# qc-tum/TNC

Hardware: NVIDIA H100
Metric: pairwise contractions/sec (effective ZGEMM TFLOP/s in zgemm_tflops) (higher is better)
Workload: dtype f64

## Files before the change

### tnc_b200/csrc/crt.cu

```cuda
#include "internal.h"
#include "sm90.h"
#include <cuda.h>
#include <algorithm>
#include <cmath>
#include <cstdio>
#include <cstdlib>

namespace tncb {

constexpr int CRT_MAX_MOD = 20;
static const int kModuli[CRT_MAX_MOD] = {256, 253, 251, 249, 247, 245, 241, 239, 233, 229,
                                         227, 223, 211, 199, 197, 193, 191, 181, 179, 173};
constexpr int CRT_BT = 128;
constexpr int CRT_BKB = WG_BKB;
#ifndef CRT_RING3_STAGES
#define CRT_RING3_STAGES 3
#endif
#ifndef CRT_RING3_BK
#define CRT_RING3_BK 128
#endif
#ifndef CRT_RING4_STAGES
#define CRT_RING4_STAGES 5
#endif
#ifndef CRT_RING4_BK
#define CRT_RING4_BK 64
#endif
template <bool KARA> struct CrtRing {
  static constexpr int STAGES = KARA ? CRT_RING3_STAGES : CRT_RING4_STAGES;
  static constexpr int BK = KARA ? CRT_RING3_BK : CRT_RING4_BK;
  using Stage = WgStage<KARA, BK>;
  static constexpr int SMEM = STAGES * Stage::BYTES + 1024;
  static_assert(SMEM <= 232448 - 1024, "stage ring exceeds the per-block shared memory of sm_90");
};
constexpr int CRT_KCHUNK_MAX = 32768;
constexpr int CRT_G = 34;

struct CrtTables {
  int nmod;
  int a_bits_a, a_bits_b;
  int mod[CRT_MAX_MOD];
  int magic[CRT_MAX_MOD];
  double inv_mod[CRT_MAX_MOD];
  double rho1[CRT_MAX_MOD];
  double rho2[CRT_MAX_MOD];
  double p_scaled;
};

double crt_log2_product(int n) {
  double s = 0;
  for (int i = 0; i < n; i++) s += std::log2((double)kModuli[i]);
  return s;
}

void crt_choose(long long K, int want_bits, int nmod_force, int* nmod, int* bits_a, int* bits_b) {
  const double lk = std::log2((double)std::max<long long>(K, 1));
  auto needed = [&](int bits) {
    int q = 2;
    while (q < CRT_MAX_MOD && crt_log2_product(q) - 1e-9 < 2.0 * bits + lk + 3.0) q++;
    return q;
  };
  int n = nmod_force > 0 ? std::min(nmod_force, needed(53)) : needed(want_bits);
  n = std::max(2, std::min(n, CRT_MAX_MOD));
  int tot = (int)std::floor(crt_log2_product(n) - lk - 3.0 - 1e-9);
  tot = std::max(tot, 2);
  int a = std::min(want_bits, tot / 2), b = std::min(want_bits, tot - a);
  *nmod = n; *bits_a = a; *bits_b = b;
}

int crt_bits_for_tolerance(long long K, double tol) {
  if (!(tol > 0.0)) return 53;
  const int a = (int)std::ceil(std::log2(16.0 * (double)std::max<long long>(K, 1) / tol));
  return std::max(8, std::min(53, a));
}

static void crt_make_tables(int nmod, int bits_a, int bits_b, CrtTables& T) {
  T.nmod = nmod; T.a_bits_a = bits_a; T.a_bits_b = bits_b;
  long double P = 1.0L;
  for (int i = 0; i < nmod; i++) P *= (long double)kModuli[i];
  for (int i = 0; i < CRT_MAX_MOD; i++) { T.mod[i] = 1; T.magic[i] = 0; T.inv_mod[i] = 1.0; T.rho1[i] = T.rho2[i] = 0.0; }
  for (int i = 0; i < nmod; i++) {
    const int m = kModuli[i];
    long long pim = 1;
    for (int j = 0; j < nmod; j++) if (j != i) pim = (pim * (kModuli[j] % m)) % m;
    long long inv = 1;
    while ((pim * inv) % m != 1) inv++;
    const unsigned long long num = (unsigned long long)inv << CRT_G;
    const unsigned long long q = num / (unsigned long long)m, rem = num % (unsigned long long)m;
    T.mod[i] = m;
    T.magic[i] = (int)std::llround(4294967296.0 / (double)m);
    T.inv_mod[i] = 1.0 / (double)m;
    T.rho1[i] = std::ldexp((double)q, -CRT_G);
    T.rho2[i] = std::ldexp((double)rem / (double)m, -CRT_G);
  }
  T.p_scaled = (double)std::ldexp(P, -(bits_a + bits_b));
}

int crt_export_tables(int nmod, int* moduli, double* rho1, double* rho2, double* log2_product) {
  CrtTables T;
  crt_make_tables(nmod, 0, 0, T);
  for (int i = 0; i < nmod; i++) {
    if (moduli) moduli[i] = T.mod[i];
    if (rho1) rho1[i] = T.rho1[i];
    if (rho2) rho2[i] = T.rho2[i];
  }
  if (log2_product) *log2_product = crt_log2_product(nmod);
  return TNCB_OK;
}

constexpr int RES_ROWS_C = 32, RES_K_C = 128;
constexpr int kExpNonFinite = 0x7fffffff;
constexpr int kExpMin = -1000;

__device__ __forceinline__ int crt_exp_from_bits(unsigned long long bits) {
  const int field = (int)(bits >> 52) & 0x7ff;
  if (field == 0x7ff) return kExpNonFinite;
  if (field == 0) return bits == 0ull ? 0 : kExpMin;
  return max(field - 1022, kExpMin);
}

__device__ __forceinline__ void crt_tile_coord(int e, int lk, int& r, int& k) {
  const int lane = e & 31, blk = e >> 5;
  const int kb = blk & ((128 >> lk) - 1), rb = blk >> (7 - lk);
  k = (kb << lk) + (lane & ((1 << lk) - 1));
  r = (rb << (5 - lk)) + (lane >> lk);
}

__global__ void __launch_bounds__(256)
crt_rowmax_kernel(const double2* __restrict__ src, const long long* __restrict__ off_row, const long long* __restrict__ off_k,
                  long long rows, long long K, int lk, unsigned long long* __restrict__ rowmax) {
  __shared__ unsigned long long s_max[RES_ROWS_C];
  __shared__ long long s_offr[RES_ROWS_C], s_offk[RES_K_C];
  const long long row0 = (long long)blockIdx.x * RES_ROWS_C, k0 = (long long)blockIdx.y * RES_K_C;
  const int tid = threadIdx.x;
  if (tid < RES_ROWS_C) { s_max[tid] = 0ull; s_offr[tid] = row0 + tid < rows ? __ldg(off_row + row0 + tid) : -1; }
  else if (tid >= 128) { const int k = tid - 128; s_offk[k] = k0 + k < K ? __ldg(off_k + k0 + k) : -1; }
  __syncthreads();
  unsigned long long mv[RES_ROWS_C * RES_K_C / 256];
#pragma unroll
  for (int it = 0; it < RES_ROWS_C * RES_K_C / 256; it++) {
    int r, k;
    crt_tile_coord(it * 256 + tid, lk, r, k);
    const long long orow = s_offr[r], ok = s_offk[k];
    mv[it] = 0ull;
    if (orow >= 0 && ok >= 0) {
      const double2 v = __ldg(src + orow + ok);
      mv[it] = max((unsigned long long)__double_as_longlong(fabs(v.x)), (unsigned long long)__double_as_longlong(fabs(v.y)));
    }
  }
  int cur_r = -1;
  unsigned long long cur_m = 0ull;
#pragma unroll
  for (int it = 0; it < RES_ROWS_C * RES_K_C / 256; it++) {
    int r, k;
    crt_tile_coord(it * 256 + tid, lk, r, k);
    unsigned long long m = mv[it];
    for (int d = 1; d < (1 << lk); d <<= 1) m = max(m, __shfl_xor_sync(0xffffffffu, m, d));
    if (r != cur_r) {
      if (cur_m && (tid & ((1 << lk) - 1)) == 0) atomicMax(&s_max[cur_r], cur_m);
      cur_r = r; cur_m = 0ull;
    }
    cur_m = max(cur_m, m);
  }
  if (cur_m && (tid & ((1 << lk) - 1)) == 0) atomicMax(&s_max[cur_r], cur_m);
  __syncthreads();
  if (tid < RES_ROWS_C && row0 + tid < rows && s_max[tid] != 0ull) atomicMax(rowmax + row0 + tid, s_max[tid]);
}

__device__ __forceinline__ int crt_fix_byte(int s, int m) {
  if (s > 127) s -= m;
  else if (s < -128) s += m;
  return s;
}
constexpr int RES_ROWS = RES_ROWS_C, RES_K = RES_K_C, RES_RS = RES_K + RES_K / 8 + 1;
template <int COMPS, bool KARA>
__global__ void __launch_bounds__(256, 3)
crt_residue_kernel(const double2* __restrict__ src, const long long* __restrict__ off_row, const long long* __restrict__ off_k,
                   long long rows, long long K, long long rowsP, long long Kp, const unsigned long long* __restrict__ rowmax, int bits, int lk,
                   const __grid_constant__ CrtTables T, int8_t* __restrict__ planes) {
  extern __shared__ __align__(16) unsigned char res_smem_raw[];
  double2* tile = reinterpret_cast<double2*>(res_smem_raw);
  __shared__ double s_scale[RES_ROWS];
  __shared__ long long s_offr[RES_ROWS], s_offk[RES_K];
  __shared__ double s_inv[CRT_MAX_MOD];
  __shared__ int s_mod[CRT_MAX_MOD];
  const long long row0 = (long long)blockIdx.x * RES_ROWS, k0 = (long long)blockIdx.y * RES_K;
  const int tid = threadIdx.x;
  const double two_a = scalbn(1.0, bits);
  if (tid >= 64 && tid < 64 + CRT_MAX_MOD) { s_inv[tid - 64] = T.inv_mod[tid - 64]; s_mod[tid - 64] = T.mod[tid - 64]; }
  if (tid < RES_ROWS) {
    const long long r = row0 + tid;
    const int e = r < rows ? crt_exp_from_bits(rowmax[r]) : 0;
    s_scale[tid] = (e == kExpNonFinite) ? 0.0 : scalbn(1.0, -e);
    s_offr[tid] = r < rows ? __ldg(off_row + r) : -1;
  } else if (tid >= 128) {
    const int k = tid - 128;
    s_offk[k] = k0 + k < K ? __ldg(off_k + k0 + k) : -1;
  }
  __syncthreads();
  double2 vv[RES_ROWS * RES_K / 256];
#pragma unroll
  for (int it = 0; it < RES_ROWS * RES_K / 256; it++) {
    int r, k;
    crt_tile_coord(it * 256 + tid, lk, r, k);
    const long long orow = s_offr[r], ok = s_offk[k];
    vv[it] = make_double2(0.0, 0.0);
    if (orow >= 0 && ok >= 0) vv[it] = __ldg(src + orow + ok);
  }
#pragma unroll
  for (int it = 0; it < RES_ROWS * RES_K / 256; it++) {
    int r, k;
    crt_tile_coord(it * 256 + tid, lk, r, k);
    const double sc = s_scale[r];
    double2 v = vv[it];
    v.x = trunc(v.x * sc * two_a);
    v.y = trunc(v.y * sc * two_a);
    if (sc == 0.0) { v.x = 0.0; v.y = 0.0; }
    tile[r * RES_RS + k + (k >> 3)] = v;
  }
  __syncthreads();
  const int r = tid >> 3;
  if (row0 + r >= rows) return;
  const double RMAGIC = 6755399441055744.0;
  const long long plane_stride = rowsP * Kp;
#pragma unroll 1
  for (int pass = 0; pass < 2; pass++) {
    const int g = (tid & 7) + 8 * pass;
    double xr[8], xi[8];
    int lr[8], li[8];
#pragma unroll
    for (int j = 0; j < 8; j++) {
      const double2 v = tile[r * RES_RS + g * 9 + j];
      xr[j] = v.x; xi[j] = v.y;
      lr[j] = (int)__double2ll_rn(v.x); li[j] = (int)__double2ll_rn(v.y);
    }
    int8_t* dst = planes + (row0 + r) * Kp + k0 + g * 8;
    const int nmod = T.nmod;
#pragma unroll 1
    for (int i = 0; i < nmod; i++) {
      const int m = s_mod[i];
      const double inv = s_inv[i];
      uint32_t wr[2] = {0, 0}, wi[2] = {0, 0}, ws[2] = {0, 0};
#pragma unroll
      for (int j = 0; j < 8; j++) {
        const int qr = __double2loint(fma(xr[j], inv, RMAGIC));
        const int qi = __double2loint(fma(xi[j], inv, RMAGIC));
        const int rr = lr[j] - qr * m, ri = li[j] - qi * m;
        constexpr uint32_t sel[4] = {0x3214u, 0x3240u, 0x3410u, 0x4210u};
        wr[j >> 2] = __byte_perm(wr[j >> 2], (uint32_t)rr, sel[j & 3]);
        wi[j >> 2] = __byte_perm(wi[j >> 2], (uint32_t)ri, sel[j & 3]);
        if (KARA) ws[j >> 2] = __byte_perm(ws[j >> 2], (uint32_t)crt_fix_byte(rr + ri, m), sel[j & 3]);
      }
      int8_t* d = dst + (long long)i * (KARA ? 3 : COMPS) * plane_stride;
      if (KARA) {
        *reinterpret_cast<uint2*>(d) = make_uint2(wr[0], wr[1]);
        *reinterpret_cast<uint2*>(d + plane_stride) = make_uint2(wi[0], wi[1]);
        *reinterpret_cast<uint2*>(d + 2 * plane_stride) = make_uint2(ws[0], ws[1]);
      } else if (COMPS == 2) {
        *reinterpret_cast<uint2*>(d) = make_uint2(wr[0], wr[1]);
        *reinterpret_cast<uint2*>(d + plane_stride) = make_uint2(wi[0], wi[1]);
      } else {
        *reinterpret_cast<uint2*>(d) = make_uint2(__vneg4(wi[0]), __vneg4(wi[1]));
        *reinterpret_cast<uint2*>(d + plane_stride) = make_uint2(wr[0], wr[1]);
        *reinterpret_cast<uint2*>(d + 2 * plane_stride) = make_uint2(wi[0], wi[1]);
      }
    }
  }
}

struct CrtGemmArgs {
  int8_t* R;
  int Np, Mp;
  int tiles_n, tiles_m, tile_m;
  int nmod, nkc, kb_per_chunk, num_kb;
  int total_items;
  int group;
  int negmod[CRT_MAX_MOD];
  int magic[CRT_MAX_MOD];
};

struct CrtItem { int mod_i, prod, kc, n0, m0; };
template <bool KARA>
__device__ __forceinline__ CrtItem crt_decode(const CrtGemmArgs& p, int item) {
  const int tiles = p.tiles_n * p.tiles_m;
  const int mk = item / tiles, t = item - mk * tiles;
  CrtItem it;
  const int mp = mk / p.nkc;
  it.kc = mk - mp * p.nkc;
  it.mod_i = KARA ? mp / 3 : mp; it.prod = KARA ? mp - it.mod_i * 3 : 0;
  const int per_band = p.group * p.tiles_m;
  const int band = t / per_band, first = band * p.group;
  const int gsize = min(p.group, p.tiles_n - first);
  const int r = t - band * per_band;
  it.n0 = (first + r % gsize) * CRT_BT;
  it.m0 = (r / gsize) * p.tile_m;
  return it;
}

template <bool KARA>
__global__ void __launch_bounds__(WG_THREADS, 1)
crt_gemm_kernel(const __grid_constant__ CUtensorMap mapB, const __grid_constant__ CUtensorMap mapA,
                const __grid_constant__ CrtGemmArgs p) {
  constexpr int STAGES = CrtRing<KARA>::STAGES, BK = CrtRing<KARA>::BK, SUB = CRT_BKB / BK;
  using Stage = typename CrtRing<KARA>::Stage;
  extern __shared__ __align__(1024) uint8_t crt_smem_raw[];
  uint8_t* smem = reinterpret_cast<uint8_t*>((reinterpret_cast<uintptr_t>(crt_smem_raw) + 1023) & ~(uintptr_t)1023);
  __shared__ uint64_t full_bar[STAGES], empty_bar[STAGES];
  const int wg = threadIdx.x >> 7, tid = threadIdx.x & 127;

  if (threadIdx.x == 0) {
    for (int s = 0; s < STAGES; s++) { wg_mbar_init(&full_bar[s], 1); wg_mbar_init(&empty_bar[s], 2); }
    asm volatile("fence.mbarrier_init.release.cluster;" ::: "memory");
  }
  __syncthreads();

  if (wg == 0) {
    wg_setmaxnreg_producer();
    if (tid != 0) return;
    int it = 0;
    for (int item = blockIdx.x; item < p.total_items; item += gridDim.x) {
      const CrtItem w = crt_decode<KARA>(p, item);
      const int kb0 = w.kc * p.kb_per_chunk, kb1 = min(p.num_kb, kb0 + p.kb_per_chunk);
      const int rowB = (KARA ? w.mod_i * 3 + w.prod : w.mod_i * 2) * p.Np + w.n0;
      const int rowA = (KARA ? w.mod_i * 3 + w.prod : w.mod_i * 3) * p.Mp + w.m0;
      for (int ks = kb0 * SUB; ks < kb1 * SUB; ks++, it++) {
        uint8_t* st = wg_produce_begin<STAGES, KARA, BK>(smem, full_bar, empty_bar, it);
        uint64_t* bar = &full_bar[it % STAGES];
        const int kx = ks * BK;
        uint8_t* a = st + Stage::A;
        wg_tma_2d(&mapB, bar, st, kx, rowB);
        if (KARA) {
          wg_tma_2d(&mapA, bar, a, kx, rowA);
          wg_tma_2d(&mapA, bar, a + Stage::TILE, kx, rowA + WG_ROWS);
        } else {
          wg_tma_2d(&mapB, bar, st + Stage::B1, kx, rowB + p.Np);
          wg_tma_2d(&mapA, bar, a, kx, rowA);
          wg_tma_2d(&mapA, bar, a + Stage::TILE, kx, rowA + p.Mp);
          wg_tma_2d(&mapA, bar, a + 2 * Stage::TILE, kx, rowA + 2 * p.Mp);
        }
      }
    }
  } else {
    wg_setmaxnreg_consumer();
    const int c = wg - 1, wq = tid >> 5, lane = tid & 31;
    const int q = lane & 3;
    const bool q0 = q & 1, q1 = q & 2;
    WgRing<STAGES, KARA, BK> ring{smem, full_bar, empty_bar};
    uint32_t acc[128];
#pragma unroll
    for (int i = 0; i < 128; i++) acc[i] = 0u;
    for (int item = blockIdx.x; item < p.total_items; item += gridDim.x) {
      const CrtItem w = crt_decode<KARA>(p, item);
      const int kb0 = w.kc * p.kb_per_chunk, kb1 = min(p.num_kb, kb0 + p.kb_per_chunk);
      bool first = true;
      for (int ks = kb0 * SUB; ks < kb1 * SUB; ks++) ring.mma_stage(acc, c, first, tid == 0);
      ring.drain(tid == 0);
      const int negm = p.negmod[w.mod_i], magic = p.magic[w.mod_i];
      int8_t* row_base[2];
#pragma unroll
      for (int h = 0; h < 2; h++) {
        const long long n = (long long)w.n0 + c * 64 + wq * 16 + (lane >> 2) + 8 * h;
        row_base[h] = KARA ? p.R + ((long long)((w.mod_i * p.nkc + w.kc) * 3 + w.prod) * p.Np + n) * p.Mp + w.m0
                           : p.R + ((long long)((w.mod_i * p.nkc + w.kc) * 2) * p.Np + n) * p.Mp + w.m0;
      }
#pragma unroll
      for (int i = 0; i < 4; i++) {
#pragma unroll
        for (int h = 0; h < 2; h++) {
          uint32_t x[4];
#pragma unroll
          for (int k = 0; k < 4; k++) {
            uint32_t u = 0;
#pragma unroll
            for (int jj = 0; jj < 2; jj++) {
#pragma unroll
              for (int e = 0; e < 2; e++) {
                const int a = (int)acc[4 * (8 * i + 2 * k + jj) + 2 * h + e];
                int t = __mulhi(a, magic) * negm + a;
                if (t > 127) t += negm;
                u |= (((uint32_t)t & 0xffu) ^ 0x80u) << (8 * (2 * jj + e));
              }
            }
            x[k] = u;
          }
          const uint32_t r0 = __shfl_xor_sync(0xffffffffu, q0 ? x[0] : x[1], 1);
          const uint32_t r1 = __shfl_xor_sync(0xffffffffu, q0 ? x[2] : x[3], 1);
          const uint32_t a0 = q0 ? r0 : x[0], a1 = q0 ? x[1] : r0;
          const uint32_t b0 = q0 ? r1 : x[2], b1 = q0 ? x[3] : r1;
          const uint32_t g0 = __shfl_xor_sync(0xffffffffu, q1 ? a0 : b0, 2);
          const uint32_t g1 = __shfl_xor_sync(0xffffffffu, q1 ? a1 : b1, 2);
          const uint32_t k0 = q1 ? b0 : a0, k1 = q1 ? b1 : a1;
          const uint32_t y0 = q1 ? g0 : k0, y1 = q1 ? g1 : k1, y2 = q1 ? k0 : g0, y3 = q1 ? k1 : g1;
          const uint4 v = make_uint4(__byte_perm(y0, y1, 0x5410), __byte_perm(y2, y3, 0x5410),
                                     __byte_perm(y0, y1, 0x7632), __byte_perm(y2, y3, 0x7632));
          const int cc = 4 * i + q;
          int8_t* dst = KARA ? row_base[h] + cc * 16
                             : row_base[h] + (i >= 2 ? (long long)p.Np * p.Mp : 0LL) + (cc & 7) * 16;
          *reinterpret_cast<uint4*>(dst) = v;
        }
      }
    }
  }
}

struct CrtReconArgs {
  const int8_t* R;
  double2* C;
  const unsigned long long* max_n;
  const unsigned long long* max_m;
  long long rows, cols, ldc;
  long long Np, Mp;
  int nkc;
};

template <bool ONE_CHUNK, bool KARA>
__global__ void __launch_bounds__(256, 4)
crt_reconstruct_kernel(const __grid_constant__ CrtReconArgs a, const __grid_constant__ CrtTables T) {
  const long long cols4 = a.Mp >> 2;
  const long long idx = (long long)blockIdx.x * blockDim.x + threadIdx.x;
  const long long n = idx / cols4, m4 = (idx - n * cols4) * 4;
  if (n >= a.rows || m4 >= a.cols) return;
  double s1r[4], s2r[4], s1i[4], s2i[4];
#pragma unroll
  for (int j = 0; j < 4; j++) { s1r[j] = s2r[j] = s1i[j] = s2i[j] = 0.0; }
  const long long plane = a.Np * a.Mp;
  const int8_t* base = a.R + n * a.Mp + m4;
  const double bias = 4503599627370496.0 + (KARA ? 256.0 : 128.0) * (double)a.nkc;
  const double bias_i = 4503599627370496.0 + (KARA ? 384.0 : 128.0) * (double)a.nkc;
#pragma unroll 8
  for (int i = 0; i < T.nmod; i++) {
    uint32_t ur[4], ui[4];
    if (KARA) {
#pragma unroll
      for (int j = 0; j < 4; j++) { ur[j] = 0; ui[j] = 0; }
      for (int c = 0; c < (ONE_CHUNK ? 1 : a.nkc); c++) {
        const int8_t* pk = base + (long long)((i * a.nkc + c) * 3) * plane;
        const uint32_t w1 = __ldg(reinterpret_cast<const uint32_t*>(pk));
        const uint32_t w2 = __ldg(reinterpret_cast<const uint32_t*>(pk + plane));
        const uint32_t w3 = __ldg(reinterpret_cast<const uint32_t*>(pk + 2 * plane));
#pragma unroll
        for (int j = 0; j < 4; j++) {
          const uint32_t k1 = __byte_perm(w1, 0, 0x4440 + j), k2 = __byte_perm(w2, 0, 0x4440 + j);
          ur[j] += 256u + k1 - k2;
          ui[j] += 512u + __byte_perm(w3, 0, 0x4440 + j) - k1 - k2;
        }
      }
    } else if (ONE_CHUNK) {
      const uint32_t wr = __ldg(reinterpret_cast<const uint32_t*>(base + (long long)(i * 2) * plane));
      const uint32_t wi = __ldg(reinterpret_cast<const uint32_t*>(base + (long long)(i * 2 + 1) * plane));
#pragma unroll
      for (int j = 0; j < 4; j++) { ur[j] = __byte_perm(wr, 0, 0x4440 + j); ui[j] = __byte_perm(wi, 0, 0x4440 + j); }
    } else {
#pragma unroll
      for (int j = 0; j < 4; j++) { ur[j] = 0; ui[j] = 0; }
      for (int c = 0; c < a.nkc; c++) {
        const int8_t* pr = base + (long long)((i * a.nkc + c) * 2) * plane;
        const uint32_t wr = __ldg(reinterpret_cast<const uint32_t*>(pr));
        const uint32_t wi = __ldg(reinterpret_cast<const uint32_t*>(pr + plane));
#pragma unroll
        for (int j = 0; j < 4; j++) { ur[j] += __byte_perm(wr, 0, 0x4440 + j); ui[j] += __byte_perm(wi, 0, 0x4440 + j); }
      }
    }
    const double r1 = T.rho1[i], r2 = T.rho2[i];
#pragma unroll
    for (int j = 0; j < 4; j++) {
      const double dr = __hiloint2double(0x43300000, (int)ur[j]) - bias;
      const double di = __hiloint2double(0x43300000, (int)ui[j]) - bias_i;
      s1r[j] = fma(dr, r1, s1r[j]); s2r[j] = fma(dr, r2, s2r[j]);
      s1i[j] = fma(di, r1, s1i[j]); s2i[j] = fma(di, r2, s2i[j]);
    }
  }
  const int en = crt_exp_from_bits(a.max_n[n]);
  double2* dst = a.C + n * a.ldc + m4;
  const double RMAGIC = 6755399441055744.0;
#pragma unroll
  for (int j = 0; j < 4; j++) {
    if (m4 + j >= a.cols) break;
    const int em = crt_exp_from_bits(a.max_m[m4 + j]);
    double2 out;
    if (en == kExpNonFinite || em == kExpNonFinite) {
      out = make_double2(__longlong_as_double(0x7ff8000000000000LL), __longlong_as_double(0x7ff8000000000000LL));
    } else {
      const double qr = ((s1r[j] + s2r[j]) + RMAGIC) - RMAGIC;
      const double qi = ((s1i[j] + s2i[j]) + RMAGIC) - RMAGIC;
      const double fr = (s1r[j] - qr) + s2r[j], fi = (s1i[j] - qi) + s2i[j];
      out = make_double2(scalbn(fr * T.p_scaled, en + em), scalbn(fi * T.p_scaled, en + em));
    }
    dst[j] = out;
  }
}

typedef CUresult (*EncodeTiledFn)(CUtensorMap*, CUtensorMapDataType, cuuint32_t, void*, const cuuint64_t*, const cuuint64_t*,
                                  const cuuint32_t*, const cuuint32_t*, CUtensorMapInterleave, CUtensorMapSwizzle,
                                  CUtensorMapL2promotion, CUtensorMapFloatOOBfill);
static EncodeTiledFn get_encode() {
  static EncodeTiledFn fn = nullptr;
  static bool tried = false;
  if (!tried) {
    tried = true;
    cudaDriverEntryPointQueryResult q;
    void* p = nullptr;
    if (cudaGetDriverEntryPoint("cuTensorMapEncodeTiled", &p, cudaEnableDefault, &q) == cudaSuccess) fn = (EncodeTiledFn)p;
  }
  return fn;
}
template <int BK>
int wg_make_map(CUtensorMap* m, void* ptr, uint64_t rows, uint64_t kbytes) {
  static_assert(BK == 128 || BK == 64, "SWIZZLE_128B or SWIZZLE_64B");
  EncodeTiledFn enc = get_encode();
  if (!enc) return fail(TNCB_ERR_CUDA, "cuTensorMapEncodeTiled is not available");
  cuuint64_t dims[2] = {kbytes, rows};
  cuuint64_t strides[1] = {kbytes};
  cuuint32_t box[2] = {(cuuint32_t)BK, (cuuint32_t)WG_ROWS};
  cuuint32_t estr[2] = {1, 1};
  CUresult r = enc(m, CU_TENSOR_MAP_DATA_TYPE_UINT8, 2, ptr, dims, strides, box, estr, CU_TENSOR_MAP_INTERLEAVE_NONE,
                   BK == 128 ? CU_TENSOR_MAP_SWIZZLE_128B : CU_TENSOR_MAP_SWIZZLE_64B, CU_TENSOR_MAP_L2_PROMOTION_L2_256B,
                   CU_TENSOR_MAP_FLOAT_OOB_FILL_NONE);
  if (r != CUDA_SUCCESS) return fail(TNCB_ERR_CUDA, "cuTensorMapEncodeTiled failed: " + std::to_string((int)r));
  return TNCB_OK;
}
template int wg_make_map<128>(CUtensorMap*, void*, uint64_t, uint64_t);
template int wg_make_map<64>(CUtensorMap*, void*, uint64_t, uint64_t);

static inline long long round_up_ll(long long x, long long a) { return (x + a - 1) / a * a; }


int launch_k1_crt(tncb_ctx* ctx, const PairPlan& P, const double2* A, const double2* B, double2* C,
                  const long long* offAm, const long long* offBn, const long long* offAk, const long long* offBk) {
  int nmod, bits_a, bits_b;
  const int want = ctx->crt_tol > 0.0 ? crt_bits_for_tolerance(P.K, ctx->crt_tol) : ctx->crt_bits;
  crt_choose(P.K, want, ctx->crt_nmod_force, &nmod, &bits_a, &bits_b);
  CrtTables T;
  crt_make_tables(nmod, bits_a, bits_b, T);
  cudaStream_t st = ctx->stream;
  const long long Kp = round_up_ll(P.K, CRT_BKB);
  const int num_kb = (int)(Kp / CRT_BKB);
  const int ctas_max = std::max(1, ctx->sm_count);
  const bool kara = ctx->crt_products == 3 || (ctx->crt_products == 0 && Kp >= ctx->crt_kara_min_k);
  const int TM = kara ? 2 * CRT_BT : CRT_BT;
  const int NPB = kara ? 3 : 2, NPR = kara ? 3 : 2;
  const long long tiles_total = round_up_ll(P.N, CRT_BT) / CRT_BT * (round_up_ll(P.M, TM) / TM);
  int nkc = (int)((Kp + CRT_KCHUNK_MAX - 1) / CRT_KCHUNK_MAX);
  {
    const long long items = tiles_total * nmod * (kara ? 3 : 1);
    const long long want = ctas_max;
    if (items * nkc < want) nkc = (int)std::min<long long>((want + items - 1) / items, std::max(1, num_kb / 8));
    nkc = std::max(1, std::min(nkc, 32));
  }
  int kb_per_chunk = (num_kb + nkc - 1) / nkc;
  nkc = (num_kb + kb_per_chunk - 1) / kb_per_chunk;
  if ((long long)kb_per_chunk * CRT_BKB > CRT_KCHUNK_MAX) return fail(TNCB_ERR_UNSUPPORTED, "K too long for the int8 engine");

  const size_t budget = ctx->crt_ws_bytes;
  long long pn = round_up_ll(P.N, CRT_BT), pm = round_up_ll(P.M, TM);
  auto ws_bytes = [&](long long n_, long long m_) {
    return (size_t)nmod * (size_t)Kp * (size_t)(NPB * n_ + 3 * m_) + (size_t)nmod * nkc * NPR * (size_t)n_ * (size_t)m_;
  };
  while (ws_bytes(pn, pm) > budget && (pm > TM || pn > CRT_BT)) {
    if (pm >= pn && pm > TM) pm = round_up_ll(pm / 2, TM);
    else if (pn > CRT_BT) pn = round_up_ll(pn / 2, CRT_BT);
    else pm = round_up_ll(pm / 2, TM);
  }
  const size_t bytesB = (size_t)nmod * NPB * pn * Kp, bytesA = (size_t)nmod * 3 * pm * Kp;
  const size_t bytesR = (size_t)nmod * nkc * NPR * pn * pm;
  const size_t bytesE = (size_t)(pn + pm) * sizeof(unsigned long long);
  void *pb = nullptr, *pa = nullptr, *pr = nullptr, *pe = nullptr;
  int rc;
  if ((rc = ctx->arena.alloc(bytesB, &pb))) return rc;
  if ((rc = ctx->arena.alloc(bytesA, &pa))) { ctx->arena.free(pb, bytesB); return rc; }
  if ((rc = ctx->arena.alloc(bytesR, &pr))) { ctx->arena.free(pb, bytesB); ctx->arena.free(pa, bytesA); return rc; }
  if ((rc = ctx->arena.alloc(bytesE, &pe))) { ctx->arena.free(pb, bytesB); ctx->arena.free(pa, bytesA); ctx->arena.free(pr, bytesR); return rc; }
  auto cleanup = [&]() { ctx->arena.free(pb, bytesB); ctx->arena.free(pa, bytesA); ctx->arena.free(pr, bytesR); ctx->arena.free(pe, bytesE); };
  unsigned long long* max_n = (unsigned long long*)pe;
  unsigned long long* max_m = max_n + pn;

  static bool attr_done_dev[64] = {false};
  bool& attr_done = attr_done_dev[ctx->device & 63];
  const int smem_gemm4 = CrtRing<false>::SMEM, smem_gemm3 = CrtRing<true>::SMEM;
  const int smem_res = RES_ROWS * RES_RS * (int)sizeof(double2);
  if (!attr_done) {
    cudaError_t e = cudaFuncSetAttribute(crt_gemm_kernel<false>, cudaFuncAttributeMaxDynamicSharedMemorySize, smem_gemm4);
    if (e == cudaSuccess) e = cudaFuncSetAttribute(crt_gemm_kernel<true>, cudaFuncAttributeMaxDynamicSharedMemorySize, smem_gemm3);
    if (e == cudaSuccess) e = cudaFuncSetAttribute(crt_residue_kernel<2, false>, cudaFuncAttributeMaxDynamicSharedMemorySize, smem_res);
    if (e == cudaSuccess) e = cudaFuncSetAttribute(crt_residue_kernel<3, false>, cudaFuncAttributeMaxDynamicSharedMemorySize, smem_res);
    if (e == cudaSuccess) e = cudaFuncSetAttribute(crt_residue_kernel<2, true>, cudaFuncAttributeMaxDynamicSharedMemorySize, smem_res);
    if (e == cudaSuccess) e = cudaFuncSetAttribute(crt_residue_kernel<3, true>, cudaFuncAttributeMaxDynamicSharedMemorySize, smem_res);
    if (e != cudaSuccess) { cleanup(); return fail(TNCB_ERR_CUDA, cudaGetErrorString(e)); }
    attr_done = true;
  }
  auto lane_split = [](const LegList& kl, bool k_is_b, const LegList& fl) {
    auto p2 = [](long long d) { int b = 0; while ((2LL << b) <= d && b < 5) b++; return b; };
    const long long ks = kl.n ? (k_is_b ? kl.sb[kl.n - 1] : kl.sa[kl.n - 1]) : (1LL << 62);
    const long long fs = fl.n ? fl.sa[fl.n - 1] : (1LL << 62);
    if (ks <= fs) return kl.n ? p2(kl.dim[kl.n - 1]) : 0;
    return 0;
  };
  const int lk_b = lane_split(P.k, true, P.n), lk_a = lane_split(P.k, false, P.m);
  ctx->last_int8_ops = 0.0; ctx->last_nmod = nmod; ctx->last_products = kara ? 3 : 4;
  bool timed = false;

  for (long long n0 = 0; n0 < P.N; n0 += pn) {
    const long long nrows = std::min(pn, P.N - n0);
    const long long Np = round_up_ll(nrows, CRT_BT);
    if (Np != nrows) cudaMemsetAsync(pb, 0, (size_t)nmod * NPB * Np * Kp, st);
    cudaMemsetAsync(max_n, 0, (size_t)nrows * sizeof(unsigned long long), st);
    {
      dim3 g((unsigned)((nrows + RES_ROWS - 1) / RES_ROWS), (unsigned)(Kp / RES_K));
      crt_rowmax_kernel<<<g, 256, 0, st>>>(B, offBn + n0, offBk, nrows, P.K, lk_b, max_n);
      if (kara) crt_residue_kernel<2, true><<<g, 256, smem_res, st>>>(B, offBn + n0, offBk, nrows, P.K, Np, Kp, max_n, bits_b, lk_b, T, (int8_t*)pb);
      else crt_residue_kernel<2, false><<<g, 256, smem_res, st>>>(B, offBn + n0, offBk, nrows, P.K, Np, Kp, max_n, bits_b, lk_b, T, (int8_t*)pb);
    }
    ctx->launches += 2;
    CUtensorMap mapB;
    if ((rc = kara ? wg_make_map<CrtRing<true>::BK>(&mapB, pb, (uint64_t)nmod * NPB * Np, (uint64_t)Kp)
                   : wg_make_map<CrtRing<false>::BK>(&mapB, pb, (uint64_t)nmod * NPB * Np, (uint64_t)Kp))) { cleanup(); return rc; }
    for (long long m0 = 0; m0 < P.M; m0 += pm) {
      const long long mcols = std::min(pm, P.M - m0);
      const long long Mp = round_up_ll(mcols, TM);
      if (Mp != mcols) cudaMemsetAsync(pa, 0, (size_t)nmod * 3 * Mp * Kp, st);
      cudaMemsetAsync(max_m, 0, (size_t)mcols * sizeof(unsigned long long), st);
      {
        dim3 g((unsigned)((mcols + RES_ROWS - 1) / RES_ROWS), (unsigned)(Kp / RES_K));
        crt_rowmax_kernel<<<g, 256, 0, st>>>(A, offAm + m0, offAk, mcols, P.K, lk_a, max_m);
        if (kara) crt_residue_kernel<3, true><<<g, 256, smem_res, st>>>(A, offAm + m0, offAk, mcols, P.K, Mp, Kp, max_m, bits_a, lk_a, T, (int8_t*)pa);
        else crt_residue_kernel<3, false><<<g, 256, smem_res, st>>>(A, offAm + m0, offAk, mcols, P.K, Mp, Kp, max_m, bits_a, lk_a, T, (int8_t*)pa);
      }
      ctx->launches += 2;
      CUtensorMap mapA;
      if ((rc = kara ? wg_make_map<CrtRing<true>::BK>(&mapA, pa, (uint64_t)nmod * 3 * Mp, (uint64_t)Kp)
                     : wg_make_map<CrtRing<false>::BK>(&mapA, pa, (uint64_t)nmod * 3 * Mp, (uint64_t)Kp))) { cleanup(); return rc; }
      CrtGemmArgs g;
      g.R = (int8_t*)pr; g.Np = (int)Np; g.Mp = (int)Mp;
      g.tiles_n = (int)(Np / CRT_BT); g.tiles_m = (int)(Mp / TM); g.tile_m = TM;
      g.nmod = nmod; g.nkc = nkc; g.kb_per_chunk = kb_per_chunk; g.num_kb = num_kb;
      const long long items = (long long)g.tiles_n * g.tiles_m * nmod * nkc * (kara ? 3 : 1);
      if (items > 0x7fffffffLL) { cleanup(); return fail(TNCB_ERR_UNSUPPORTED, "too many work items"); }
      g.total_items = (int)items;
      g.group = ctx->crt_group;
      for (int i = 0; i < CRT_MAX_MOD; i++) { g.negmod[i] = -T.mod[i]; g.magic[i] = T.magic[i]; }
      const unsigned grid = (unsigned)std::min<long long>(ctas_max, items);
      const double ops = 2.0 * (kara ? 3.0 : 4.0) * (double)nmod * (double)Np * (double)Mp * (double)Kp;
      const bool time_this = ctx->time_gemm == 2 || (ctx->time_gemm == 1 && !timed);
      if (time_this) gemm_timer_begin(ctx);
      if (kara) crt_gemm_kernel<true><<<grid, WG_THREADS, smem_gemm3, st>>>(mapB, mapA, g);
      else crt_gemm_kernel<false><<<grid, WG_THREADS, smem_gemm4, st>>>(mapB, mapA, g);
      cudaError_t e = cudaGetLastError();
      if (time_this) { gemm_timer_end(ctx, ops); timed = true; }
      if (e != cudaSuccess) { cleanup(); return fail(TNCB_ERR_CUDA, std::string("crt_gemm_kernel launch: ") + cudaGetErrorString(e)); }
      ctx->last_int8_ops += ops;
      CrtReconArgs r;
      r.R = (const int8_t*)pr; r.C = C + n0 * P.M + m0; r.max_n = max_n; r.max_m = max_m;
      r.rows = nrows; r.cols = mcols; r.ldc = P.M; r.Np = Np; r.Mp = Mp; r.nkc = nkc;
      const long long threads = nrows * (Mp / 4);
      const unsigned rg = (unsigned)((threads + 255) / 256);
      if (kara) {
        if (nkc == 1) crt_reconstruct_kernel<true, true><<<rg, 256, 0, st>>>(r, T);
        else crt_reconstruct_kernel<false, true><<<rg, 256, 0, st>>>(r, T);
      } else {
        if (nkc == 1) crt_reconstruct_kernel<true, false><<<rg, 256, 0, st>>>(r, T);
        else crt_reconstruct_kernel<false, false><<<rg, 256, 0, st>>>(r, T);
      }
      ctx->launches += 2;
    }
  }
  ctx->engine_count[4]++;
  cudaError_t e = cudaGetLastError();
  cleanup();
  if (e != cudaSuccess) return fail(TNCB_ERR_CUDA, std::string("K1' (CRT) launch: ") + cudaGetErrorString(e));
  return TNCB_OK;
}

}
```

Baseline: 5853.

## Restructure CRT residue and reconstruct kernels with cp.async staging and wider stores

The residue kernel now stages an 8x512 input tile into shared memory with cp.async, and each thread handles 16 consecutive k elements so residues go out as 16-byte stores instead of 8-byte ones. It also drops the padding memsets by covering the whole padded row range, and walks k tiles in reverse order. The single-chunk reconstruct kernel now stages each row segment's residue planes into shared memory with cp.async before decoding, in place of scattered __ldg loads. The changes aim to cut memory-transaction overhead in the pre- and post-processing around the int8 GEMM, at the cost of more shared memory per block and lower occupancy.

```diff
diff --git a/tnc_b200/csrc/crt.cu b/tnc_b200/csrc/crt.cu
--- a/tnc_b200/csrc/crt.cu
+++ b/tnc_b200/csrc/crt.cu
@@ -171,98 +171,109 @@
   else if (s < -128) s += m;
   return s;
 }
-constexpr int RES_ROWS = RES_ROWS_C, RES_K = RES_K_C, RES_RS = RES_K + RES_K / 8 + 1;
+constexpr int RES_R = 8, RES_KT = 512, RES_THREADS = 256;
+constexpr int RES_RS = RES_KT + RES_KT / 16 + 4;
+constexpr int RES_SMEM = RES_R * RES_RS * (int)sizeof(double2);
+
+static __device__ __forceinline__ void crt_cp_async16(unsigned smem_addr, const void* gptr, bool pred) {
+  asm volatile("cp.async.cg.shared.global [%0], [%1], 16, %2;\n" ::"r"(smem_addr), "l"(gptr), "r"(pred ? 16 : 0));
+}
+
 template <int COMPS, bool KARA>
-__global__ void __launch_bounds__(256, 3)
+__global__ void __launch_bounds__(RES_THREADS, 2)
 crt_residue_kernel(const double2* __restrict__ src, const long long* __restrict__ off_row, const long long* __restrict__ off_k,
-                   long long rows, long long K, long long rowsP, long long Kp, const unsigned long long* __restrict__ rowmax, int bits, int lk,
-                   const __grid_constant__ CrtTables T, int8_t* __restrict__ planes) {
+                   long long rows, long long K, long long rowsP, long long Kp, const unsigned long long* __restrict__ rowmax, int bits,
+                   int lk, const __grid_constant__ CrtTables T, int8_t* __restrict__ planes) {
   extern __shared__ __align__(16) unsigned char res_smem_raw[];
   double2* tile = reinterpret_cast<double2*>(res_smem_raw);
-  __shared__ double s_scale[RES_ROWS];
-  __shared__ long long s_offr[RES_ROWS], s_offk[RES_K];
+  __shared__ long long s_offr[RES_R], s_offk[RES_KT];
+  __shared__ double s_scale[RES_R];
   __shared__ double s_inv[CRT_MAX_MOD];
   __shared__ int s_mod[CRT_MAX_MOD];
-  const long long row0 = (long long)blockIdx.x * RES_ROWS, k0 = (long long)blockIdx.y * RES_K;
-  const int tid = threadIdx.x;
-  const double two_a = scalbn(1.0, bits);
-  if (tid >= 64 && tid < 64 + CRT_MAX_MOD) { s_inv[tid - 64] = T.inv_mod[tid - 64]; s_mod[tid - 64] = T.mod[tid - 64]; }
-  if (tid < RES_ROWS) {
+  const long long row0 = (long long)blockIdx.x * RES_R, k0 = (long long)(gridDim.y - 1 - blockIdx.y) * RES_KT;
+  const int tid = threadIdx.x, warp = tid >> 5, lane = tid & 31;
+  if (tid < CRT_MAX_MOD) { s_inv[tid] = T.inv_mod[tid]; s_mod[tid] = T.mod[tid]; }
+  if (tid < RES_R) {
     const long long r = row0 + tid;
     const int e = r < rows ? crt_exp_from_bits(rowmax[r]) : 0;
     s_scale[tid] = (e == kExpNonFinite) ? 0.0 : scalbn(1.0, -e);
     s_offr[tid] = r < rows ? __ldg(off_row + r) : -1;
-  } else if (tid >= 128) {
-    const int k = tid - 128;
-    s_offk[k] = k0 + k < K ? __ldg(off_k + k0 + k) : -1;
-  }
+  }
+  for (int k = tid; k < RES_KT; k += RES_THREADS) s_offk[k] = k0 + k < K ? __ldg(off_k + k0 + k) : -1;
   __syncthreads();
-  double2 vv[RES_ROWS * RES_K / 256];
-#pragma unroll
-  for (int it = 0; it < RES_ROWS * RES_K / 256; it++) {
-    int r, k;
-    crt_tile_coord(it * 256 + tid, lk, r, k);
-    const long long orow = s_offr[r], ok = s_offk[k];
-    vv[it] = make_double2(0.0, 0.0);
-    if (orow >= 0 && ok >= 0) vv[it] = __ldg(src + orow + ok);
-  }
-#pragma unroll
-  for (int it = 0; it < RES_ROWS * RES_K / 256; it++) {
-    int r, k;
-    crt_tile_coord(it * 256 + tid, lk, r, k);
-    const double sc = s_scale[r];
-    double2 v = vv[it];
-    v.x = trunc(v.x * sc * two_a);
-    v.y = trunc(v.y * sc * two_a);
-    if (sc == 0.0) { v.x = 0.0; v.y = 0.0; }
-    tile[r * RES_RS + k + (k >> 3)] = v;
+  {
+    const int lq = max(lk, 2);
+    const unsigned sbase = (unsigned)__cvta_generic_to_shared(tile);
+#pragma unroll
+    for (int it = 0; it < RES_R * RES_KT / RES_THREADS; it++) {
+      const int e = it * RES_THREADS + tid, blk = e >> 5;
+      const int kb = blk & ((RES_KT >> lq) - 1), rb = blk >> (9 - lq);
+      const int k = (kb << lq) + (lane & ((1 << lq) - 1)), r = (rb << (5 - lq)) + (lane >> lq);
+      const long long orow = s_offr[r], ok = s_offk[k];
+      const bool valid = orow >= 0 && ok >= 0;
+      crt_cp_async16(sbase + (unsigned)(r * RES_RS + k + (k >> 4)) * 16u, valid ? src + orow + ok : src, valid);
+    }
+    asm volatile("cp.async.commit_group;\ncp.async.wait_group 0;\n" ::: "memory");
   }
   __syncthreads();
-  const int r = tid >> 3;
-  if (row0 + r >= rows) return;
-  const double RMAGIC = 6755399441055744.0;
-  const long long plane_stride = rowsP * Kp;
-#pragma unroll 1
-  for (int pass = 0; pass < 2; pass++) {
-    const int g = (tid & 7) + 8 * pass;
-    double xr[8], xi[8];
-    int lr[8], li[8];
-#pragma unroll
-    for (int j = 0; j < 8; j++) {
-      const double2 v = tile[r * RES_RS + g * 9 + j];
-      xr[j] = v.x; xi[j] = v.y;
-      lr[j] = (int)__double2ll_rn(v.x); li[j] = (int)__double2ll_rn(v.y);
-    }
-    int8_t* dst = planes + (row0 + r) * Kp + k0 + g * 8;
+  const int r = warp, kl = lane * 16;
+  double2 v[16];
+#pragma unroll
+  for (int j = 0; j < 16; j++) v[j] = tile[r * RES_RS + kl + lane + j];
+  const double sc = s_scale[r];
+  const double two_a = scalbn(1.0, bits);
+  double xr[16], xi[16];
+  int lr[16], li[16];
+#pragma unroll
+  for (int j = 0; j < 16; j++) {
+    double2 w = v[j];
+    w.x = trunc(w.x * sc * two_a);
+    w.y = trunc(w.y * sc * two_a);
+    if (sc == 0.0) { w.x = 0.0; w.y = 0.0; }
+    xr[j] = w.x; xi[j] = w.y;
+    lr[j] = (int)__double2ll_rn(w.x); li[j] = (int)__double2ll_rn(w.y);
+  }
+  const long long kk = k0 + kl;
+  if (kk < Kp) {
+    const double RMAGIC = 6755399441055744.0;
+    const long long plane_stride = rowsP * Kp;
+    int8_t* dst = planes + (row0 + r) * Kp + kk;
     const int nmod = T.nmod;
 #pragma unroll 1
     for (int i = 0; i < nmod; i++) {
-      const int m = s_mod[i];
+      const int md = s_mod[i];
       const double inv = s_inv[i];
-      uint32_t wr[2] = {0, 0}, wi[2] = {0, 0}, ws[2] = {0, 0};
-#pragma unroll
-      for (int j = 0; j < 8; j++) {
+      uint32_t wr[4] = {0, 0, 0, 0}, wi[4] = {0, 0, 0, 0};
+#pragma unroll
+      for (int j = 0; j < 16; j++) {
         const int qr = __double2loint(fma(xr[j], inv, RMAGIC));
         const int qi = __double2loint(fma(xi[j], inv, RMAGIC));
-        const int rr = lr[j] - qr * m, ri = li[j] - qi * m;
+        const int rr = lr[j] - qr * md, ri = li[j] - qi * md;
         constexpr uint32_t sel[4] = {0x3214u, 0x3240u, 0x3410u, 0x4210u};
         wr[j >> 2] = __byte_perm(wr[j >> 2], (uint32_t)rr, sel[j & 3]);
         wi[j >> 2] = __byte_perm(wi[j >> 2], (uint32_t)ri, sel[j & 3]);
-        if (KARA) ws[j >> 2] = __byte_perm(ws[j >> 2], (uint32_t)crt_fix_byte(rr + ri, m), sel[j & 3]);
       }
-      int8_t* d = dst + (long long)i * (KARA ? 3 : COMPS) * plane_stride;
+      int8_t* d = dst;
       if (KARA) {
-        *reinterpret_cast<uint2*>(d) = make_uint2(wr[0], wr[1]);
-        *reinterpret_cast<uint2*>(d + plane_stride) = make_uint2(wi[0], wi[1]);
-        *reinterpret_cast<uint2*>(d + 2 * plane_stride) = make_uint2(ws[0], ws[1]);
+        *reinterpret_cast<uint4*>(d) = make_uint4(wr[0], wr[1], wr[2], wr[3]);
+        *reinterpret_cast<uint4*>(d + plane_stride) = make_uint4(wi[0], wi[1], wi[2], wi[3]);
+        uint32_t ws[4] = {0, 0, 0, 0};
+#pragma unroll
+        for (int j = 0; j < 16; j++) {
+          const int rr = (int)(int8_t)(wr[j >> 2] >> (8 * (j & 3))), ri = (int)(int8_t)(wi[j >> 2] >> (8 * (j & 3)));
+          constexpr uint32_t sel[4] = {0x3214u, 0x3240u, 0x3410u, 0x4210u};
+          ws[j >> 2] = __byte_perm(ws[j >> 2], (uint32_t)crt_fix_byte(rr + ri, md), sel[j & 3]);
+        }
+        *reinterpret_cast<uint4*>(d + 2 * plane_stride) = make_uint4(ws[0], ws[1], ws[2], ws[3]);
       } else if (COMPS == 2) {
-        *reinterpret_cast<uint2*>(d) = make_uint2(wr[0], wr[1]);
-        *reinterpret_cast<uint2*>(d + plane_stride) = make_uint2(wi[0], wi[1]);
+        *reinterpret_cast<uint4*>(d) = make_uint4(wr[0], wr[1], wr[2], wr[3]);
+        *reinterpret_cast<uint4*>(d + plane_stride) = make_uint4(wi[0], wi[1], wi[2], wi[3]);
       } else {
-        *reinterpret_cast<uint2*>(d) = make_uint2(__vneg4(wi[0]), __vneg4(wi[1]));
-        *reinterpret_cast<uint2*>(d + plane_stride) = make_uint2(wr[0], wr[1]);
-        *reinterpret_cast<uint2*>(d + 2 * plane_stride) = make_uint2(wi[0], wi[1]);
+        *reinterpret_cast<uint4*>(d) = make_uint4(__vneg4(wi[0]), __vneg4(wi[1]), __vneg4(wi[2]), __vneg4(wi[3]));
+        *reinterpret_cast<uint4*>(d + plane_stride) = make_uint4(wr[0], wr[1], wr[2], wr[3]);
+        *reinterpret_cast<uint4*>(d + 2 * plane_stride) = make_uint4(wi[0], wi[1], wi[2], wi[3]);
       }
+      dst += (KARA ? 3 : COMPS) * plane_stride;
     }
   }
 }
@@ -412,18 +423,46 @@
   int nkc;
 };
 
+constexpr int RECON_THREADS = 256, RECON_SEG = 4 * RECON_THREADS;
 template <bool ONE_CHUNK, bool KARA>
-__global__ void __launch_bounds__(256, 4)
+__global__ void __launch_bounds__(RECON_THREADS, 4)
 crt_reconstruct_kernel(const __grid_constant__ CrtReconArgs a, const __grid_constant__ CrtTables T) {
-  const long long cols4 = a.Mp >> 2;
-  const long long idx = (long long)blockIdx.x * blockDim.x + threadIdx.x;
-  const long long n = idx / cols4, m4 = (idx - n * cols4) * 4;
-  if (n >= a.rows || m4 >= a.cols) return;
+  extern __shared__ __align__(16) unsigned char rec_smem[];
+  long long n, m4, plane;
+  const int8_t* base;
+  if (ONE_CHUNK) {
+    const long long segs = (a.cols + RECON_SEG - 1) / RECON_SEG;
+    n = blockIdx.x / segs;
+    const long long m0 = (blockIdx.x - n * segs) * RECON_SEG;
+    const int cpr = (int)(min((long long)RECON_SEG, a.cols - m0) + 15) >> 4;
+    const int nruns = T.nmod * (KARA ? 3 : 2);
+    const int8_t* g = a.R + n * a.Mp + m0;
+    const long long gplane = a.Np * a.Mp;
+    const unsigned sbase = (unsigned)__cvta_generic_to_shared(rec_smem);
+    for (int c = threadIdx.x; c < nruns * cpr; c += RECON_THREADS) {
+      const int p = c / cpr, o = (c - p * cpr) * 16;
+      crt_cp_async16(sbase + (unsigned)(p * RECON_SEG + o), g + p * gplane + o, true);
+    }
+    asm volatile("cp.async.commit_group;\ncp.async.wait_group 0;\n" ::: "memory");
+    __syncthreads();
+    m4 = m0 + 4 * threadIdx.x;
+    if (m4 >= a.cols) return;
+    base = reinterpret_cast<const int8_t*>(rec_smem) + 4 * threadIdx.x;
+    plane = RECON_SEG;
+  } else {
+    const long long cols4 = a.Mp >> 2;
+    const long long idx = (long long)blockIdx.x * blockDim.x + threadIdx.x;
+    n = idx / cols4; m4 = (idx - n * cols4) * 4;
+    if (n >= a.rows || m4 >= a.cols) return;
+    base = a.R + n * a.Mp + m4;
+    plane = a.Np * a.Mp;
+  }
+  auto ld = [&](const int8_t* p) {
+    return ONE_CHUNK ? *reinterpret_cast<const uint32_t*>(p) : __ldg(reinterpret_cast<const uint32_t*>(p));
+  };
   double s1r[4], s2r[4], s1i[4], s2i[4];
 #pragma unroll
   for (int j = 0; j < 4; j++) { s1r[j] = s2r[j] = s1i[j] = s2i[j] = 0.0; }
-  const long long plane = a.Np * a.Mp;
-  const int8_t* base = a.R + n * a.Mp + m4;
   const double bias = 4503599627370496.0 + (KARA ? 256.0 : 128.0) * (double)a.nkc;
   const double bias_i = 4503599627370496.0 + (KARA ? 384.0 : 128.0) * (double)a.nkc;
 #pragma unroll 8
@@ -434,9 +473,7 @@
       for (int j = 0; j < 4; j++) { ur[j] = 0; ui[j] = 0; }
       for (int c = 0; c < (ONE_CHUNK ? 1 : a.nkc); c++) {
         const int8_t* pk = base + (long long)((i * a.nkc + c) * 3) * plane;
-        const uint32_t w1 = __ldg(reinterpret_cast<const uint32_t*>(pk));
-        const uint32_t w2 = __ldg(reinterpret_cast<const uint32_t*>(pk + plane));
-        const uint32_t w3 = __ldg(reinterpret_cast<const uint32_t*>(pk + 2 * plane));
+        const uint32_t w1 = ld(pk), w2 = ld(pk + plane), w3 = ld(pk + 2 * plane);
 #pragma unroll
         for (int j = 0; j < 4; j++) {
           const uint32_t k1 = __byte_perm(w1, 0, 0x4440 + j), k2 = __byte_perm(w2, 0, 0x4440 + j);
@@ -445,8 +482,7 @@
         }
       }
     } else if (ONE_CHUNK) {
-      const uint32_t wr = __ldg(reinterpret_cast<const uint32_t*>(base + (long long)(i * 2) * plane));
-      const uint32_t wi = __ldg(reinterpret_cast<const uint32_t*>(base + (long long)(i * 2 + 1) * plane));
+      const uint32_t wr = ld(base + (long long)(i * 2) * plane), wi = ld(base + (long long)(i * 2 + 1) * plane);
 #pragma unroll
       for (int j = 0; j < 4; j++) { ur[j] = __byte_perm(wr, 0, 0x4440 + j); ui[j] = __byte_perm(wi, 0, 0x4440 + j); }
     } else {
@@ -576,14 +612,15 @@
   static bool attr_done_dev[64] = {false};
   bool& attr_done = attr_done_dev[ctx->device & 63];
   const int smem_gemm4 = CrtRing<false>::SMEM, smem_gemm3 = CrtRing<true>::SMEM;
-  const int smem_res = RES_ROWS * RES_RS * (int)sizeof(double2);
   if (!attr_done) {
     cudaError_t e = cudaFuncSetAttribute(crt_gemm_kernel<false>, cudaFuncAttributeMaxDynamicSharedMemorySize, smem_gemm4);
     if (e == cudaSuccess) e = cudaFuncSetAttribute(crt_gemm_kernel<true>, cudaFuncAttributeMaxDynamicSharedMemorySize, smem_gemm3);
-    if (e == cudaSuccess) e = cudaFuncSetAttribute(crt_residue_kernel<2, false>, cudaFuncAttributeMaxDynamicSharedMemorySize, smem_res);
-    if (e == cudaSuccess) e = cudaFuncSetAttribute(crt_residue_kernel<3, false>, cudaFuncAttributeMaxDynamicSharedMemorySize, smem_res);
-    if (e == cudaSuccess) e = cudaFuncSetAttribute(crt_residue_kernel<2, true>, cudaFuncAttributeMaxDynamicSharedMemorySize, smem_res);
-    if (e == cudaSuccess) e = cudaFuncSetAttribute(crt_residue_kernel<3, true>, cudaFuncAttributeMaxDynamicSharedMemorySize, smem_res);
+    if (e == cudaSuccess) e = cudaFuncSetAttribute(crt_residue_kernel<2, false>, cudaFuncAttributeMaxDynamicSharedMemorySize, RES_SMEM);
+    if (e == cudaSuccess) e = cudaFuncSetAttribute(crt_residue_kernel<3, false>, cudaFuncAttributeMaxDynamicSharedMemorySize, RES_SMEM);
+    if (e == cudaSuccess) e = cudaFuncSetAttribute(crt_residue_kernel<2, true>, cudaFuncAttributeMaxDynamicSharedMemorySize, RES_SMEM);
+    if (e == cudaSuccess) e = cudaFuncSetAttribute(crt_residue_kernel<3, true>, cudaFuncAttributeMaxDynamicSharedMemorySize, RES_SMEM);
+    if (e == cudaSuccess) e = cudaFuncSetAttribute(crt_reconstruct_kernel<true, false>, cudaFuncAttributeMaxDynamicSharedMemorySize, CRT_MAX_MOD * 2 * RECON_SEG);
+    if (e == cudaSuccess) e = cudaFuncSetAttribute(crt_reconstruct_kernel<true, true>, cudaFuncAttributeMaxDynamicSharedMemorySize, CRT_MAX_MOD * 3 * RECON_SEG);
     if (e != cudaSuccess) { cleanup(); return fail(TNCB_ERR_CUDA, cudaGetErrorString(e)); }
     attr_done = true;
   }
@@ -595,36 +632,32 @@
     return 0;
   };
   const int lk_b = lane_split(P.k, true, P.n), lk_a = lane_split(P.k, false, P.m);
+  auto prepare = [&](const double2* src, const long long* off_row, const long long* off_k, long long rows, long long rowsP,
+                     int bits, int lk, unsigned long long* rowmax, int8_t* planes, bool bt) {
+    cudaMemsetAsync(rowmax, 0, (size_t)rows * sizeof(unsigned long long), st);
+    crt_rowmax_kernel<<<dim3((unsigned)((rows + RES_ROWS_C - 1) / RES_ROWS_C), (unsigned)(Kp / RES_K_C)), 256, 0, st>>>(
+        src, off_row, off_k, rows, P.K, lk, rowmax);
+    const dim3 g((unsigned)(rowsP / RES_R), (unsigned)((Kp + RES_KT - 1) / RES_KT));
+    if (kara && bt) crt_residue_kernel<2, true><<<g, RES_THREADS, RES_SMEM, st>>>(src, off_row, off_k, rows, P.K, rowsP, Kp, rowmax, bits, lk, T, planes);
+    else if (kara) crt_residue_kernel<3, true><<<g, RES_THREADS, RES_SMEM, st>>>(src, off_row, off_k, rows, P.K, rowsP, Kp, rowmax, bits, lk, T, planes);
+    else if (bt) crt_residue_kernel<2, false><<<g, RES_THREADS, RES_SMEM, st>>>(src, off_row, off_k, rows, P.K, rowsP, Kp, rowmax, bits, lk, T, planes);
+    else crt_residue_kernel<3, false><<<g, RES_THREADS, RES_SMEM, st>>>(src, off_row, off_k, rows, P.K, rowsP, Kp, rowmax, bits, lk, T, planes);
+    ctx->launches += 2;
+  };
   ctx->last_int8_ops = 0.0; ctx->last_nmod = nmod; ctx->last_products = kara ? 3 : 4;
   bool timed = false;
 
   for (long long n0 = 0; n0 < P.N; n0 += pn) {
     const long long nrows = std::min(pn, P.N - n0);
     const long long Np = round_up_ll(nrows, CRT_BT);
-    if (Np != nrows) cudaMemsetAsync(pb, 0, (size_t)nmod * NPB * Np * Kp, st);
-    cudaMemsetAsync(max_n, 0, (size_t)nrows * sizeof(unsigned long long), st);
-    {
-      dim3 g((unsigned)((nrows + RES_ROWS - 1) / RES_ROWS), (unsigned)(Kp / RES_K));
-      crt_rowmax_kernel<<<g, 256, 0, st>>>(B, offBn + n0, offBk, nrows, P.K, lk_b, max_n);
-      if (kara) crt_residue_kernel<2, true><<<g, 256, smem_res, st>>>(B, offBn + n0, offBk, nrows, P.K, Np, Kp, max_n, bits_b, lk_b, T, (int8_t*)pb);
-      else crt_residue_kernel<2, false><<<g, 256, smem_res, st>>>(B, offBn + n0, offBk, nrows, P.K, Np, Kp, max_n, bits_b, lk_b, T, (int8_t*)pb);
-    }
-    ctx->launches += 2;
+    prepare(B, offBn + n0, offBk, nrows, Np, bits_b, lk_b, max_n, (int8_t*)pb, true);
     CUtensorMap mapB;
     if ((rc = kara ? wg_make_map<CrtRing<true>::BK>(&mapB, pb, (uint64_t)nmod * NPB * Np, (uint64_t)Kp)
                    : wg_make_map<CrtRing<false>::BK>(&mapB, pb, (uint64_t)nmod * NPB * Np, (uint64_t)Kp))) { cleanup(); return rc; }
     for (long long m0 = 0; m0 < P.M; m0 += pm) {
       const long long mcols = std::min(pm, P.M - m0);
       const long long Mp = round_up_ll(mcols, TM);
-      if (Mp != mcols) cudaMemsetAsync(pa, 0, (size_t)nmod * 3 * Mp * Kp, st);
-      cudaMemsetAsync(max_m, 0, (size_t)mcols * sizeof(unsigned long long), st);
-      {
-        dim3 g((unsigned)((mcols + RES_ROWS - 1) / RES_ROWS), (unsigned)(Kp / RES_K));
-        crt_rowmax_kernel<<<g, 256, 0, st>>>(A, offAm + m0, offAk, mcols, P.K, lk_a, max_m);
-        if (kara) crt_residue_kernel<3, true><<<g, 256, smem_res, st>>>(A, offAm + m0, offAk, mcols, P.K, Mp, Kp, max_m, bits_a, lk_a, T, (int8_t*)pa);
-        else crt_residue_kernel<3, false><<<g, 256, smem_res, st>>>(A, offAm + m0, offAk, mcols, P.K, Mp, Kp, max_m, bits_a, lk_a, T, (int8_t*)pa);
-      }
-      ctx->launches += 2;
+      prepare(A, offAm + m0, offAk, mcols, Mp, bits_a, lk_a, max_m, (int8_t*)pa, false);
       CUtensorMap mapA;
       if ((rc = kara ? wg_make_map<CrtRing<true>::BK>(&mapA, pa, (uint64_t)nmod * 3 * Mp, (uint64_t)Kp)
                      : wg_make_map<CrtRing<false>::BK>(&mapA, pa, (uint64_t)nmod * 3 * Mp, (uint64_t)Kp))) { cleanup(); return rc; }
@@ -650,14 +683,15 @@
       CrtReconArgs r;
       r.R = (const int8_t*)pr; r.C = C + n0 * P.M + m0; r.max_n = max_n; r.max_m = max_m;
       r.rows = nrows; r.cols = mcols; r.ldc = P.M; r.Np = Np; r.Mp = Mp; r.nkc = nkc;
-      const long long threads = nrows * (Mp / 4);
-      const unsigned rg = (unsigned)((threads + 255) / 256);
-      if (kara) {
-        if (nkc == 1) crt_reconstruct_kernel<true, true><<<rg, 256, 0, st>>>(r, T);
-        else crt_reconstruct_kernel<false, true><<<rg, 256, 0, st>>>(r, T);
+      if (nkc == 1) {
+        const unsigned rg = (unsigned)(nrows * ((mcols + RECON_SEG - 1) / RECON_SEG));
+        const int smem = nmod * NPR * RECON_SEG;
+        if (kara) crt_reconstruct_kernel<true, true><<<rg, RECON_THREADS, smem, st>>>(r, T);
+        else crt_reconstruct_kernel<true, false><<<rg, RECON_THREADS, smem, st>>>(r, T);
       } else {
-        if (nkc == 1) crt_reconstruct_kernel<true, false><<<rg, 256, 0, st>>>(r, T);
-        else crt_reconstruct_kernel<false, false><<<rg, 256, 0, st>>>(r, T);
+        const unsigned rg = (unsigned)((nrows * (Mp / 4) + RECON_THREADS - 1) / RECON_THREADS);
+        if (kara) crt_reconstruct_kernel<false, true><<<rg, RECON_THREADS, 0, st>>>(r, T);
+        else crt_reconstruct_kernel<false, false><<<rg, RECON_THREADS, 0, st>>>(r, T);
       }
       ctx->launches += 2;
     }
```

New measurement: 6142 (median of 6 runs). 1.05x the previous value.
